# ORNL/DDStore

Measured on AMD Instinct MI355X. Metric: samples/sec (global-shuffle sample fetch), higher is better.
Workload: dtype bf16; 1 GPU; model=store-globalshuffle-fetch, global_batch=262144, rows_per_rank=2097152, row_bytes=512, store_dtype=f32, parallelism=dp1, mode=fetch

## Files before the change

### ddstore_amd/csrc/ddstore_kernels.hip

```cpp

#include "ddstore_kernels.h"

#include <hip/hip_fp16.h>
#include <hip/hip_bf16.h>
#include <hip/hip_fp8.h>
#include <type_traits>
#include <cstdlib>
#include <string>

namespace ddstore {

namespace {

constexpr int kBlock = 256;
constexpr int64_t kMaxBlocks = 32768;

inline int n_blocks(int64_t work_items) {
    int64_t b = (work_items + kBlock - 1) / kBlock;
    if (b < 1) b = 1;
    if (b > kMaxBlocks) b = kMaxBlocks;
    return (int)b;
}

template <typename T, int N>
struct alignas(sizeof(T) * N) VecT {
    T v[N];
};

__device__ __forceinline__ int owner_of(const int64_t* prefix, int nparts, int64_t row) {
    int lo = 0, hi = nparts - 1;
    while (lo < hi) {
        int mid = (lo + hi + 1) >> 1;
        if (prefix[mid] <= row) lo = mid; else hi = mid - 1;
    }
    return lo;
}

template <typename P, int NPFX = 1>
struct LdsDir {
    int64_t prefix[NPFX][DDS_MAX_PARTS + 1];
    P base[DDS_MAX_PARTS];

    __device__ __forceinline__ void load(const void* const* peer_base, int nparts,
                                         const int64_t* gprefix0,
                                         const int64_t* gprefix1 = nullptr) {
        for (int i = threadIdx.x; i <= nparts; i += kBlock) {
            prefix[0][i] = gprefix0[i];
            if constexpr (NPFX == 2) prefix[1][i] = gprefix1[i];
        }
        for (int i = threadIdx.x; i < nparts; i += kBlock)
            base[i] = reinterpret_cast<P>(peer_base[i]);
        __syncthreads();
    }
};

template <typename P, int NPFX>
__device__ __forceinline__ int owner_of(const LdsDir<P, NPFX>& d, int nparts, int64_t row) {
    return owner_of(d.prefix[0], nparts, row);
}

template <typename P, int NPFX>
__device__ __forceinline__ bool out_of_range(const LdsDir<P, NPFX>& d, int nparts,
                                             int64_t g) {
    return g < 0 || g >= d.prefix[0][nparts];
}

template <typename T>
constexpr bool is_fp8_v =
    std::is_same_v<T, __hip_fp8_e4m3> || std::is_same_v<T, __hip_fp8_e5m2>;

__device__ __forceinline__ float f64_to_f32(double v) {
#pragma clang fp contract(off)
    return static_cast<float>(v);
}

template <typename Tout, typename Tin>
__device__ __forceinline__ Tout cvt(Tin v) {
    if constexpr (std::is_same_v<Tout, Tin>) {
        return v;
    } else if constexpr (std::is_same_v<Tin, double> &&
                         (std::is_same_v<Tout, __half> ||
                          std::is_same_v<Tout, __hip_bfloat16>)) {
        return cvt<Tout, float>(f64_to_f32(v));
    } else if constexpr (std::is_same_v<Tout, uint8_t> &&
                         std::is_floating_point_v<Tin>) {
        return static_cast<uint8_t>(static_cast<int32_t>(v));
    } else if constexpr (std::is_same_v<Tin, __half>) {
        return cvt<Tout, float>(__half2float(v));
    } else if constexpr (std::is_same_v<Tin, __hip_bfloat16>) {
        return cvt<Tout, float>(__bfloat162float(v));
    } else if constexpr (is_fp8_v<Tin>) {
        return cvt<Tout, float>(static_cast<float>(v));
    } else if constexpr (std::is_same_v<Tout, __half>) {
        return __float2half(static_cast<float>(v));
    } else if constexpr (std::is_same_v<Tout, __hip_bfloat16>) {
        return __float2bfloat16(static_cast<float>(v));
    } else if constexpr (is_fp8_v<Tout>) {
        const float f = static_cast<float>(v);
        Tout r(f);
        if constexpr (std::is_same_v<Tout, __hip_fp8_e4m3>) {
            if (fabsf(f) > 464.0f) r.__x = 0x7F;
        } else {
            if (fabsf(f) >= 61440.0f) r.__x = f < 0.0f ? 0xFC : 0x7C;
        }
        return r;
    } else {
        return static_cast<Tout>(v);
    }
}

struct XfIdentity {
    static constexpr bool kNeedsCol = false;
    template <typename Tout, typename Tin>
    __device__ __forceinline__ Tout apply(Tin v) const { return v; }
};
struct XfCast {
    static constexpr bool kNeedsCol = false;
    template <typename Tout, typename Tin>
    __device__ __forceinline__ Tout apply(Tin v) const { return cvt<Tout>(v); }
};
struct XfAffine {
    static constexpr bool kNeedsCol = false;
    float scale, shift;
    uint32_t opaque_zero = 0;
    template <typename Tout, typename Tin>
    __device__ __forceinline__ Tout apply(Tin v) const {
        float y = fmaf(cvt<float>(v), scale, shift);
        if constexpr (std::is_same_v<Tout, __half>)
            y = __uint_as_float(__float_as_uint(y) | opaque_zero);
        return cvt<Tout>(y);
    }
};
struct XfAffineCol {
    static constexpr bool kNeedsCol = true;
    const float* scale;
    const float* shift;
    uint32_t opaque_zero = 0;
    template <typename Tout, typename Tin>
    __device__ __forceinline__ Tout apply(Tin v, float sc, float sh) const {
        float y = fmaf(cvt<float>(v), sc, sh);
        if constexpr (std::is_same_v<Tout, __half>)
            y = __uint_as_float(__float_as_uint(y) | opaque_zero);
        return cvt<Tout>(y);
    }
};

template <typename Tout, int VEC, bool CONTIG, typename Xf, typename Tin>
__device__ __forceinline__ void xf_chunk(const Xf& xf, const float* sc, const float* sh,
                                         const VecT<Tin, VEC>& vin, VecT<Tout, VEC>& vout,
                                         uint32_t col0, uint32_t disp = 0) {
    if constexpr (!Xf::kNeedsCol) {
#pragma unroll
        for (int k = 0; k < VEC; ++k) vout.v[k] = xf.template apply<Tout>(vin.v[k]);
    } else if constexpr (CONTIG) {
        const VecT<float, VEC> s = *reinterpret_cast<const VecT<float, VEC>*>(sc + col0);
        const VecT<float, VEC> h = *reinterpret_cast<const VecT<float, VEC>*>(sh + col0);
#pragma unroll
        for (int k = 0; k < VEC; ++k)
            vout.v[k] = xf.template apply<Tout>(vin.v[k], s.v[k], h.v[k]);
    } else {
        uint32_t cc = col0;
#pragma unroll
        for (int k = 0; k < VEC; ++k) {
            vout.v[k] = xf.template apply<Tout>(vin.v[k], sc[cc], sh[cc]);
            cc = cc + 1 == disp ? 0 : cc + 1;
        }
    }
}

template <typename Tin, typename Tout, int VEC, typename Xf>
__global__ void __launch_bounds__(kBlock)
k_gather_oneshot(const void* const* peer_base, const int64_t* gprefix, int nparts,
                 const int64_t* idx, int64_t nidx, int64_t row_elems, Xf xf,
                 Tout* __restrict__ out, unsigned long long* oob) {
    using Vin = VecT<Tin, VEC>;
    using Vout = VecT<Tout, VEC>;
    __shared__ LdsDir<const Tin*> dir;
    dir.load(peer_base, nparts, gprefix);

    const int64_t cpr = row_elems / VEC;
    const int64_t total = nidx * cpr;
    for (int64_t t = (int64_t)blockIdx.x * kBlock + threadIdx.x; t < total;
         t += (int64_t)gridDim.x * kBlock) {
        const int64_t r = t / cpr;
        const int64_t c = t - r * cpr;
        const int64_t g = idx[r];
        if (out_of_range(dir, nparts, g)) {
            if (c == 0) atomicAdd(oob, 1ull);
            continue;
        }
        const int p = owner_of(dir, nparts, g);
        const Vin vin = *reinterpret_cast<const Vin*>(
            dir.base[p] + (g - dir.prefix[0][p]) * row_elems + c * VEC);
        Vout vout;
        if constexpr (Xf::kNeedsCol)
            xf_chunk<Tout, VEC, true>(xf, xf.scale, xf.shift, vin, vout,
                                      (uint32_t)c * VEC);
        else
            xf_chunk<Tout, VEC, true>(xf, nullptr, nullptr, vin, vout, 0u);
        *reinterpret_cast<Vout*>(out + t * VEC) = vout;
    }
}

typedef uint32_t dds_u32x4 __attribute__((ext_vector_type(4)));
typedef uint32_t dds_u32x2 __attribute__((ext_vector_type(2)));
#define DDS_GLOBAL_AS __attribute__((address_space(1)))

template <typename V>
__device__ __forceinline__ void store_out(V* p, const V& v) {
    static_assert(sizeof(V) == 16, "store side is exactly 16 B per lane");
    dds_u32x4 w;
    __builtin_memcpy(&w, &v, 16);
    __builtin_nontemporal_store(w, reinterpret_cast<dds_u32x4*>(p));
}

template <typename V>
__device__ __forceinline__ V load_global(uintptr_t a) {
    constexpr int B = sizeof(V);
    V r;
    if constexpr (B % 16 == 0) {
        dds_u32x4 w[B / 16];
#pragma unroll
        for (int i = 0; i < B / 16; ++i)
            w[i] = ((const DDS_GLOBAL_AS dds_u32x4*)a)[i];
        __builtin_memcpy(&r, w, B);
    } else if constexpr (B == 8) {
        const dds_u32x2 w = *(const DDS_GLOBAL_AS dds_u32x2*)a;
        __builtin_memcpy(&r, &w, B);
    } else if constexpr (B == 4) {
        const uint32_t w = *(const DDS_GLOBAL_AS uint32_t*)a;
        __builtin_memcpy(&r, &w, B);
    } else {
        static_assert(B == 2, "unsupported vector size");
        const uint16_t w = *(const DDS_GLOBAL_AS uint16_t*)a;
        __builtin_memcpy(&r, &w, B);
    }
    return r;
}

template <int INB>
constexpr int tiled_unroll() {
    return INB >= 128 ? 1 : (128 / INB > 8 ? 8 : 128 / INB);
}

template <typename Xf, int VEC, int U, bool = Xf::kNeedsCol>
struct TiledCols {};
template <typename Xf, int VEC, int U>
struct TiledCols<Xf, VEC, U, true> {
    VecT<float, VEC> s[U], h[U];
};

template <typename Tin, typename Tout, typename Xf, bool LDSDIR>
__global__ void __launch_bounds__(kBlock)
k_gather_tiled(const GatherDirK dir, const void* const* peer_base,
               const int64_t* gprefix, int nparts,
               const int64_t* __restrict__ idx, int64_t nidx, int64_t ntiles,
               uint32_t cpr, uint32_t tile_rows, Xf xf,
               Tout* __restrict__ out, unsigned long long* oob) {
    constexpr int VEC = 16 / sizeof(Tout);
    constexpr int INB = VEC * sizeof(Tin);
    constexpr int U = tiled_unroll<INB>();
    using Vin = VecT<Tin, VEC>;
    using Vout = VecT<Tout, VEC>;
    __shared__ LdsDir<uintptr_t> ldir;
    if constexpr (LDSDIR) ldir.load(peer_base, nparts, gprefix);
    const int64_t total = LDSDIR ? ldir.prefix[0][nparts] : dir.prefix[DDS_DIR_KPARTS];
    TiledCols<Xf, VEC, U> tc;

    const uint32_t lane = threadIdx.x & 63;
    const uint32_t wave = __builtin_amdgcn_readfirstlane(threadIdx.x >> 6);
    const int64_t wstride = (int64_t)gridDim.x * (kBlock / 64);
    int64_t tile = (int64_t)blockIdx.x * (kBlock / 64) + wave;
    if (tile >= ntiles) return;

    const uint32_t q64 = 64u / cpr, r64 = 64u % cpr;
    const uint32_t rl0 = lane / cpr, c0 = lane - rl0 * cpr;
    const int64_t row_bytes = (int64_t)cpr * INB;

    int64_t g_next = 0;
    {
        const int64_t r = tile * tile_rows + lane;
        if (lane < tile_rows && r < nidx) g_next = idx[r];
    }
    for (; tile < ntiles; tile += wstride) {
        const int64_t row0 = tile * tile_rows;
        const int64_t left = nidx - row0;
        const uint32_t nrows = left < (int64_t)tile_rows ? (uint32_t)left : tile_rows;
        const int64_t g = g_next;
        if (tile + wstride < ntiles) {
            const int64_t r = (tile + wstride) * tile_rows + lane;
            if (lane < tile_rows && r < nidx) g_next = idx[r];
        }
        uintptr_t src = 0;
        if (lane < nrows) {
            if (g < 0 || g >= total) {
                atomicAdd(oob, 1ull);
            } else if constexpr (LDSDIR) {
                const int p = owner_of(ldir, nparts, g);
                src = ldir.base[p] + (uintptr_t)((g - ldir.prefix[0][p]) * row_bytes);
            } else {
                int64_t pf = dir.prefix[0];
                uintptr_t bs = reinterpret_cast<uintptr_t>(dir.base[0]);
#pragma unroll
                for (int k = 1; k < DDS_DIR_KPARTS; ++k) {
                    const bool ge = dir.prefix[k] <= g;
                    pf = ge ? dir.prefix[k] : pf;
                    bs = ge ? reinterpret_cast<uintptr_t>(dir.base[k]) : bs;
                }
                src = bs + (uintptr_t)((g - pf) * row_bytes);
            }
        }
        Vout* __restrict__ op = reinterpret_cast<Vout*>(out) + row0 * cpr;
        const uint32_t nch = nrows * cpr;
        const bool clean = __ballot(lane < nrows && src == 0) == 0;
        uint32_t rl = rl0, c = c0;
        for (uint32_t jb = 0; jb < nch; jb += 64u * U) {
            if (clean && jb + 64u * U <= nch) {
                Vin vin[U];
#pragma unroll
                for (int u = 0; u < U; ++u) {
                    const uintptr_t sp =
                        (uintptr_t)__shfl((unsigned long long)src, (int)(rl & 63u));
                    if constexpr (Xf::kNeedsCol) {
                        tc.s[u] = *reinterpret_cast<const VecT<float, VEC>*>(xf.scale + c * VEC);
                        tc.h[u] = *reinterpret_cast<const VecT<float, VEC>*>(xf.shift + c * VEC);
                    }
                    vin[u] = load_global<Vin>(sp + (uintptr_t)(c * (uint32_t)INB));
                    c += r64;
                    rl += q64;
                    if (c >= cpr) {
                        c -= cpr;
                        rl += 1;
                    }
                }
#pragma unroll
                for (int u = 0; u < U; ++u) {
                    Vout vout;
                    if constexpr (Xf::kNeedsCol) {
#pragma unroll
                        for (int k = 0; k < VEC; ++k)
                            vout.v[k] = xf.template apply<Tout>(vin[u].v[k], tc.s[u].v[k],
                                                                tc.h[u].v[k]);
                    } else {
#pragma unroll
                        for (int k = 0; k < VEC; ++k)
                            vout.v[k] = xf.template apply<Tout>(vin[u].v[k]);
                    }
                    store_out(&op[jb + 64u * u + lane], vout);
                }
            } else {
#pragma unroll 1
                for (int u = 0; u < U; ++u) {
                    const uint32_t j = jb + 64u * u + lane;
                    const uintptr_t sp =
                        (uintptr_t)__shfl((unsigned long long)src, (int)(rl & 63u));
                    if (j < nch && sp != 0) {
                        const Vin v =
                            load_global<Vin>(sp + (uintptr_t)(c * (uint32_t)INB));
                        Vout vout;
                        if constexpr (Xf::kNeedsCol) {
                            xf_chunk<Tout, VEC, true>(xf, xf.scale, xf.shift, v, vout,
                                                      c * (uint32_t)VEC);
                        } else {
#pragma unroll
                            for (int k = 0; k < VEC; ++k)
                                vout.v[k] = xf.template apply<Tout>(v.v[k]);
                        }
                        store_out(&op[j], vout);
                    }
                    c += r64;
                    rl += q64;
                    if (c >= cpr) {
                        c -= cpr;
                        rl += 1;
                    }
                }
            }
        }
    }
}

__global__ void __launch_bounds__(kBlock)
k_csr_lens(const int64_t* goff, const int64_t* idx, int64_t nidx, int64_t nsamples,
           int64_t* __restrict__ lens, unsigned long long* oob,
           unsigned long long* elems) {
    int64_t acc = 0;
    for (int64_t i = (int64_t)blockIdx.x * kBlock + threadIdx.x; i < nidx;
         i += (int64_t)gridDim.x * kBlock) {
        const int64_t g = idx[i];
        if (g < 0 || g >= nsamples) {
            lens[i] = 0;
            if (oob) atomicAdd(oob, 1ull);
            continue;
        }
        const int64_t L = goff[g + 1] - goff[g];
        lens[i] = L;
        acc += L;
    }
    if (elems) {
        for (int off = 32; off > 0; off >>= 1) acc += __shfl_down(acc, off);
        if ((threadIdx.x & 63) == 0 && acc)
            atomicAdd(elems, (unsigned long long)acc);
    }
}

__device__ __forceinline__ void copy_dwords_store16(
    uint32_t* __restrict__ dst, const uint32_t* __restrict__ src,
    int64_t nd, int tid, int nthreads) {
    const int64_t h_align = (int64_t)((4 - ((((uintptr_t)dst) >> 2) & 3)) & 3);
    const int64_t h = h_align < nd ? h_align : nd;
    for (int64_t i = tid; i < h; i += nthreads) dst[i] = src[i];
    const int64_t nb = (nd - h) >> 2;
    uint4* d4 = reinterpret_cast<uint4*>(dst + h);
    const uint32_t* s2 = src + h;
    for (int64_t i = tid; i < nb; i += nthreads) {
        uint4 o;
        o.x = s2[4 * i];
        o.y = s2[4 * i + 1];
        o.z = s2[4 * i + 2];
        o.w = s2[4 * i + 3];
        d4[i] = o;
    }
    for (int64_t i = h + (nb << 2) + tid; i < nd; i += nthreads) dst[i] = src[i];
}

template <typename U>
__device__ __forceinline__ void copy_units(U* dst, const U* src, int64_t n, int tid,
                                           int nthreads) {
    if constexpr (std::is_same_v<U, uint32_t>) {
        copy_dwords_store16(dst, src, n, tid, nthreads);
    } else {
        for (int64_t c = tid; c < n; c += nthreads) dst[c] = src[c];
    }
}

template <typename U, int GROUP>
__global__ void __launch_bounds__(kBlock)
k_gather_csr_wave(const void* const* peer_base,
                  const int64_t* sample_prefix, const int64_t* elem_prefix, int nparts,
                  const int64_t* goff,
                  const int64_t* idx, int64_t nidx,
                  const int64_t* out_off, int64_t units_per_elem,
                  int64_t cap_elems,
                  U* __restrict__ out, unsigned long long* ctrs) {
    __shared__ LdsDir<const U*, 2> dir;
    dir.load(peer_base, nparts, sample_prefix, elem_prefix);

    constexpr int GPB = kBlock / GROUP;
    const int64_t first = (int64_t)blockIdx.x * GPB + threadIdx.x / GROUP;
    const int64_t step = (int64_t)gridDim.x * GPB;
    const int tid = threadIdx.x % GROUP;
    for (int64_t s = first; s < nidx; s += step) {
        const int64_t g = idx[s];
        if (out_of_range(dir, nparts, g)) {
            if (tid == 0) atomicAdd(ctrs + DDS_CTR_OOB, 1ull);
            continue;
        }
        const int p = owner_of(dir, nparts, g);
        const int64_t e0 = goff[g];
        const int64_t len = goff[g + 1] - e0;
        const int64_t o0 = out_off[s];
        if (len <= 0) continue;
        if (o0 < 0 || o0 + len > cap_elems) {
            if (tid == 0) {
                atomicAdd(ctrs + DDS_CTR_CAP, 1ull);
                atomicAdd(ctrs + DDS_CTR_ELEMS,
                          (unsigned long long)(-(long long)len));
            }
            continue;
        }
        copy_units<U>(out + o0 * units_per_elem,
                      dir.base[p] + (e0 - dir.prefix[1][p]) * units_per_elem,
                      len * units_per_elem, tid, GROUP);
    }
}

constexpr int kItemBytes = 1024;

__device__ __forceinline__ void block_scan_pair(int64_t& x, int64_t& y,
                                                int64_t* s_wsum2, int lane,
                                                int wave, int64_t* tile_tot) {
    for (int off = 1; off < 64; off <<= 1) {
        int64_t ax = __shfl_up(x, off);
        int64_t ay = __shfl_up(y, off);
        if (lane >= off) {
            x += ax;
            y += ay;
        }
    }
    if (lane == 63) {
        s_wsum2[2 * wave] = x;
        s_wsum2[2 * wave + 1] = y;
    }
    __syncthreads();
    if (threadIdx.x == 0) {
        int64_t ax = 0, ay = 0;
        for (int w = 0; w < kBlock / 64; ++w) {
            int64_t tx = s_wsum2[2 * w], ty = s_wsum2[2 * w + 1];
            s_wsum2[2 * w] = ax;
            s_wsum2[2 * w + 1] = ay;
            ax += tx;
            ay += ty;
        }
        if (tile_tot) {
            tile_tot[0] = ax;
            tile_tot[1] = ay;
        }
    }
    __syncthreads();
    x += s_wsum2[2 * wave];
    y += s_wsum2[2 * wave + 1];
}

__global__ void __launch_bounds__(kBlock)
k_csr_plan1(const int64_t* goff, int64_t nsamples,
            const int64_t* idx, int64_t nidx, int64_t item_elems,
            int64_t* __restrict__ lens_tmp, int64_t* __restrict__ e0_tmp,
            int64_t* __restrict__ aggs, unsigned long long* ctrs) {
    __shared__ int64_t s_wsum2[2 * (kBlock / 64)];
    __shared__ int64_t s_tot[2];
    const int lane = threadIdx.x & 63;
    const int wave = threadIdx.x >> 6;
    const int64_t ntiles = (nidx + kBlock - 1) / kBlock;
    for (int64_t tile = blockIdx.x; tile < ntiles; tile += gridDim.x) {
        const int64_t i = tile * kBlock + threadIdx.x;
        int64_t L = 0, e0 = -1;
        if (i < nidx) {
            const int64_t g = idx[i];
            if (g < 0 || g >= nsamples) {
                atomicAdd(ctrs + DDS_CTR_OOB, 1ull);
            } else {
                e0 = goff[g];
                L = goff[g + 1] - e0;
            }
            lens_tmp[i] = L;
            e0_tmp[i] = e0;
        }
        int64_t x = L;
        int64_t y = L > 0 ? (L + item_elems - 1) / item_elems : 0;
        block_scan_pair(x, y, s_wsum2, lane, wave, s_tot);
        if (threadIdx.x == 0) {
            aggs[2 * tile] = s_tot[0];
            aggs[2 * tile + 1] = s_tot[1];
        }
        __syncthreads();
    }
}

__global__ void __launch_bounds__(kBlock)
k_csr_plan2(int64_t* __restrict__ aggs, int64_t ntiles,
            int64_t* __restrict__ meta, unsigned long long* ctrs) {
    __shared__ int64_t s_wsum2[2 * (kBlock / 64)];
    __shared__ int64_t s_tot[2];
    __shared__ int64_t s_carry[2];
    const int lane = threadIdx.x & 63;
    const int wave = threadIdx.x >> 6;
    if (threadIdx.x == 0) {
        s_carry[0] = 0;
        s_carry[1] = 0;
    }
    __syncthreads();
    for (int64_t base = 0; base < ntiles; base += kBlock) {
        const int64_t t = base + threadIdx.x;
        int64_t x = t < ntiles ? aggs[2 * t] : 0;
        int64_t y = t < ntiles ? aggs[2 * t + 1] : 0;
        const int64_t mx = x, my = y;
        block_scan_pair(x, y, s_wsum2, lane, wave, s_tot);
        if (t < ntiles) {
            aggs[2 * t] = s_carry[0] + x - mx;
            aggs[2 * t + 1] = s_carry[1] + y - my;
        }
        __syncthreads();
        if (threadIdx.x == 0) {
            s_carry[0] += s_tot[0];
            s_carry[1] += s_tot[1];
        }
        __syncthreads();
    }
    if (threadIdx.x == 0) {
        meta[0] = s_carry[1];
        meta[1] = s_carry[0];
        atomicAdd(ctrs + DDS_CTR_ELEMS, (unsigned long long)s_carry[0]);
    }
}

static_assert(DDS_MAX_PARTS <= 128,
              "the owner travels as p << 56 in a signed 64-bit descriptor and comes "
              "back as (int)(d0 >> 56): 127 is the largest owner that keeps it "
              "non-negative");
__global__ void __launch_bounds__(kBlock)
k_csr_plan3(const int64_t* __restrict__ lens_tmp,
            const int64_t* __restrict__ e0_tmp, int64_t nidx,
            const int64_t* sample_prefix, const int64_t* elem_prefix,
            int nparts, const int64_t* idx,
            int64_t item_elems, int64_t units_per_elem, int64_t cap_elems,
            const int64_t* __restrict__ aggs,
            int64_t* __restrict__ out_off,
            int64_t* __restrict__ desc, int64_t desc_cap,
            unsigned long long* ctrs) {
    __shared__ int64_t s_wsum2[2 * (kBlock / 64)];
    __shared__ int64_t s_sprefix[DDS_MAX_PARTS + 1];
    __shared__ int64_t s_eprefix[DDS_MAX_PARTS + 1];
    for (int i = threadIdx.x; i <= nparts; i += kBlock) {
        s_sprefix[i] = sample_prefix[i];
        s_eprefix[i] = elem_prefix[i];
    }
    __syncthreads();
    const int lane = threadIdx.x & 63;
    const int wave = threadIdx.x >> 6;
    const int64_t ntiles = (nidx + kBlock - 1) / kBlock;
    for (int64_t tile = blockIdx.x; tile < ntiles; tile += gridDim.x) {
        const int64_t i = tile * kBlock + threadIdx.x;
        const int64_t L = i < nidx ? lens_tmp[i] : 0;
        int64_t x = L;
        int64_t items = L > 0 ? (L + item_elems - 1) / item_elems : 0;
        int64_t y = items;
        block_scan_pair(x, y, s_wsum2, lane, wave, nullptr);
        const int64_t e_base = aggs[2 * tile], i_base = aggs[2 * tile + 1];
        if (i < nidx) {
            const int64_t excl_e = e_base + x - L;
            const int64_t excl_i = i_base + y - items;
            out_off[i + 1] = e_base + x;
            if (i == 0) out_off[0] = 0;
            if (L > 0) {
                if (excl_e + L > cap_elems ||
                    excl_i + items > desc_cap ||
                    L * units_per_elem >= (int64_t(1) << 44)) {
                    atomicAdd(ctrs + DDS_CTR_CAP, 1ull);
                    atomicAdd(ctrs + DDS_CTR_ELEMS,
                              (unsigned long long)(-(long long)L));
                    const int64_t end =
                        items < desc_cap - excl_i ? excl_i + items : desc_cap;
                    for (int64_t j = excl_i; j < end; ++j) {
                        desc[2 * j] = 0;
                        desc[2 * j + 1] = 0;
                    }
                } else {
                    const int64_t g = idx[i];
                    const int64_t p = owner_of(s_sprefix, nparts, g);
                    const int64_t src0 =
                        (e0_tmp[i] - s_eprefix[p]) * units_per_elem;
                    const int64_t dst0 = excl_e * units_per_elem;
                    const int64_t iu = item_elems * units_per_elem;
                    const int64_t nu = L * units_per_elem;
                    for (int64_t k = 0; k < items; ++k) {
                        const int64_t off = k * iu;
                        const int64_t n = nu - off < iu ? nu - off : iu;
                        desc[2 * (excl_i + k)] = (p << 56) | (src0 + off);
                        desc[2 * (excl_i + k) + 1] = (n << 44) | (dst0 + off);
                    }
                }
            }
        }
        __syncthreads();
    }
}

template <typename U, int GROUP>
__global__ void __launch_bounds__(kBlock)
k_gather_csr_items(const void* const* peer_base, int nparts,
                   const int64_t* __restrict__ desc,
                   const int64_t* __restrict__ meta, int64_t desc_cap,
                   U* __restrict__ out) {
    __shared__ const U* s_base[DDS_MAX_PARTS];
    for (int i = threadIdx.x; i < nparts; i += kBlock)
        s_base[i] = reinterpret_cast<const U*>(peer_base[i]);
    __syncthreads();
    const int64_t total = meta[0] < desc_cap ? meta[0] : desc_cap;
    constexpr int GPB = kBlock / GROUP;
    const int64_t first = (int64_t)blockIdx.x * GPB + threadIdx.x / GROUP;
    const int64_t step = (int64_t)gridDim.x * GPB;
    const int tid = threadIdx.x % GROUP;
    for (int64_t j = first; j < total; j += step) {
        const int64_t d0 = desc[2 * j];
        const int64_t d1 = desc[2 * j + 1];
        const int p = (int)(d0 >> 56);
        const int64_t src_u = d0 & ((int64_t(1) << 56) - 1);
        const int64_t n_u = d1 >> 44;
        const int64_t dst_u = d1 & ((int64_t(1) << 44) - 1);
        copy_units<U>(out + dst_u, s_base[p] + src_u, n_u, tid, GROUP);
    }
}

constexpr int kPadCountBlocks = 64;

template <typename P>
__device__ __forceinline__ void count_padded(const LdsDir<P, 2>& dir, int nparts,
                                             const int64_t* goff, const int64_t* idx,
                                             int64_t nidx, int64_t max_len,
                                             unsigned long long* s_acc,
                                             unsigned long long* ctrs) {
    const int64_t nb = gridDim.x < (unsigned)kPadCountBlocks ? gridDim.x : kPadCountBlocks;
    unsigned long long acc_elems = 0, acc_oob = 0;
    for (int64_t i = (int64_t)blockIdx.x * kBlock + threadIdx.x; i < nidx;
         i += nb * kBlock) {
        const int64_t g = idx[i];
        if (out_of_range(dir, nparts, g)) {
            acc_oob += 1;
        } else {
            const int64_t len = goff[g + 1] - goff[g];
            acc_elems += (unsigned long long)(len < max_len ? len : max_len);
        }
    }
    for (int off = 32; off > 0; off >>= 1) {
        acc_elems += __shfl_down(acc_elems, off);
        acc_oob += __shfl_down(acc_oob, off);
    }
    if ((threadIdx.x & 63) == 0) {
        s_acc[2 * (threadIdx.x >> 6)] = acc_elems;
        s_acc[2 * (threadIdx.x >> 6) + 1] = acc_oob;
    }
    __syncthreads();
    if (threadIdx.x == 0) {
        unsigned long long e = 0, o = 0;
        for (int w = 0; w < kBlock / 64; ++w) {
            e += s_acc[2 * w];
            o += s_acc[2 * w + 1];
        }
        if (e) atomicAdd(ctrs + DDS_CTR_ELEMS, e);
        if (o) atomicAdd(ctrs + DDS_CTR_OOB, o);
    }
}

template <typename Tin, typename Tout, int VEC, typename Xf>
__global__ void __launch_bounds__(kBlock)
k_gather_csr_padded(const void* const* peer_base, const int64_t* sample_prefix,
                    const int64_t* elem_prefix, int nparts, const int64_t* goff,
                    const int64_t* idx, int64_t nidx, int64_t disp, int64_t max_len,
                    int lg_group, bool aligned, Xf xf, dds_u32x4 pad16,
                    Tout* __restrict__ out, int64_t* __restrict__ lengths,
                    unsigned long long* ctrs) {
    using Vin = VecT<Tin, VEC>;
    using Vout = VecT<Tout, VEC>;
    static_assert(sizeof(Vout) <= 16, "pad16 covers one output chunk");
    __shared__ LdsDir<const Tin*, 2> dir;
    __shared__ unsigned long long s_acc[2 * (kBlock / 64)];
    dir.load(peer_base, nparts, sample_prefix, elem_prefix);

    Vout vpad;
    __builtin_memcpy(&vpad, &pad16, sizeof(Vout));
    const int group = 1 << lg_group;
    const int tid = threadIdx.x & (group - 1);
    const int64_t first =
        (int64_t)blockIdx.x * (kBlock >> lg_group) + (threadIdx.x >> lg_group);
    const int64_t step = (int64_t)gridDim.x * (kBlock >> lg_group);
    const int64_t row_elems = max_len * disp;
    const int64_t cpr = row_elems / VEC;
    const float* csc = nullptr;
    const float* csh = nullptr;
    uint32_t d32 = 0, col0 = 0, cstep = 0;
    if constexpr (Xf::kNeedsCol) {
        csc = xf.scale;
        csh = xf.shift;
        d32 = (uint32_t)disp;
        col0 = (uint32_t)(((uint32_t)tid * (uint32_t)VEC) % d32);
        cstep = (uint32_t)(((uint32_t)group * (uint32_t)VEC) % d32);
    }
    if (blockIdx.x < kPadCountBlocks)
        count_padded(dir, nparts, goff, idx, nidx, max_len, s_acc, ctrs);
    for (int64_t s = first; s < nidx; s += step) {
        const int64_t g = idx[s];
        const Tin* sp = nullptr;
        int64_t nvalid = 0;
        if (out_of_range(dir, nparts, g)) {
            if (tid == 0) lengths[s] = 0;
        } else {
            const int p = owner_of(dir, nparts, g);
            const int64_t e0 = goff[g];
            const int64_t len = goff[g + 1] - e0;
            const int64_t take = len < max_len ? len : max_len;
            sp = dir.base[p] + (e0 - dir.prefix[1][p]) * disp;
            nvalid = take * disp;
            if (tid == 0) lengths[s] = len;
        }
        Vout* __restrict__ op = reinterpret_cast<Vout*>(out + s * row_elems);
        uint32_t col = col0;
        for (int64_t c = tid; c < cpr; c += group) {
            const int64_t e = c * VEC;
            Vout vout = vpad;
            if (e < nvalid) {
                if (VEC == 1 || aligned) {
                    const Vin vin = *reinterpret_cast<const Vin*>(sp + e);
                    xf_chunk<Tout, VEC, true>(xf, csc, csh, vin, vout, col);
                } else if (e + VEC <= nvalid) {
                    Vin x;
#pragma unroll
                    for (int k = 0; k < VEC; ++k) x.v[k] = sp[e + k];
                    xf_chunk<Tout, VEC, false>(xf, csc, csh, x, vout, col, d32);
                } else {
                    uint32_t cc = col;
#pragma unroll
                    for (int k = 0; k < VEC; ++k) {
                        if (e + k < nvalid) {
                            if constexpr (Xf::kNeedsCol)
                                vout.v[k] = xf.template apply<Tout>(sp[e + k], csc[cc],
                                                                    csh[cc]);
                            else
                                vout.v[k] = xf.template apply<Tout>(sp[e + k]);
                        }
                        if constexpr (Xf::kNeedsCol) cc = cc + 1 == d32 ? 0 : cc + 1;
                    }
                }
            }
            op[c] = vout;
            if constexpr (Xf::kNeedsCol) {
                col += cstep;
                if (col >= d32) col -= d32;
            }
        }
    }
}


__global__ void __launch_bounds__(kBlock)
k_csr_scan3(const int64_t* __restrict__ lens_tmp, int64_t nidx,
            const int64_t* __restrict__ aggs, int64_t* __restrict__ out_off) {
    __shared__ int64_t s_wsum2[2 * (kBlock / 64)];
    const int lane = threadIdx.x & 63;
    const int wave = threadIdx.x >> 6;
    const int64_t ntiles = (nidx + kBlock - 1) / kBlock;
    for (int64_t tile = blockIdx.x; tile < ntiles; tile += gridDim.x) {
        const int64_t i = tile * kBlock + threadIdx.x;
        int64_t x = i < nidx ? lens_tmp[i] : 0;
        int64_t y = 0;
        block_scan_pair(x, y, s_wsum2, lane, wave, nullptr);
        if (i < nidx) {
            out_off[i + 1] = aggs[2 * tile] + x;
            if (i == 0) out_off[0] = 0;
        }
        __syncthreads();
    }
}

template <typename T>
struct IdPair {
    T src, dst;
};

constexpr int kGraphGroup = 64;

template <typename Tin, typename Tout, int GROUP, bool COO>
__global__ void __launch_bounds__(kBlock)
k_gather_csr_relabel(const void* const* peer_base, const int64_t* sample_prefix,
                     const int64_t* elem_prefix, int nparts, const int64_t* goff,
                     const int64_t* idx, int64_t nidx,
                     const int64_t* __restrict__ ptr,
                     const int64_t* __restrict__ edge_ptr, int64_t ncap,
                     int64_t ecap, Tout* __restrict__ out,
                     unsigned long long* ctrs) {
    using Pin = VecT<Tin, 2>;
    __shared__ LdsDir<const Pin*, 2> dir;
    dir.load(peer_base, nparts, sample_prefix, elem_prefix);

    constexpr int GPB = kBlock / GROUP;
    const int64_t first = (int64_t)blockIdx.x * GPB + threadIdx.x / GROUP;
    const int64_t step = (int64_t)gridDim.x * GPB;
    const int tid = threadIdx.x % GROUP;
    for (int64_t s = first; s < nidx; s += step) {
        const int64_t g = idx[s];
        if (out_of_range(dir, nparts, g)) continue;
        const int64_t o0 = edge_ptr[s];
        const int64_t len = edge_ptr[s + 1] - o0;
        if (len <= 0) continue;
        if (ptr[s + 1] > ncap || o0 < 0 || o0 + len > ecap) {
            if (tid == 0) {
                atomicAdd(ctrs + DDS_CTR_CAP, 1ull);
                atomicAdd(ctrs + DDS_CTR_ELEMS, (unsigned long long)(-(long long)len));
            }
            continue;
        }
        const Tout shift = static_cast<Tout>(ptr[s]);
        const int p = owner_of(dir, nparts, g);
        const Pin* __restrict__ sp = dir.base[p] + (goff[g] - dir.prefix[1][p]);
        for (int64_t e = tid; e < len; e += GROUP) {
            const Pin v = sp[e];
            const Tout a = static_cast<Tout>(v.v[0]) + shift;
            const Tout b = static_cast<Tout>(v.v[1]) + shift;
            if constexpr (COO) {
                out[o0 + e] = a;
                out[ecap + o0 + e] = b;
            } else {
                reinterpret_cast<IdPair<Tout>*>(out)[o0 + e] = IdPair<Tout>{a, b};
            }
        }
    }
}

template <typename T>
__device__ __forceinline__ void fill_store16(T* __restrict__ dst, int64_t n, T val,
                                             int64_t tid, int64_t nthreads) {
    constexpr int V = 16 / sizeof(T);
    using Vt = VecT<T, V>;
    const int64_t h_align =
        (int64_t)(((16 - ((uintptr_t)dst & 15)) & 15) / sizeof(T));
    const int64_t h = h_align < n ? h_align : n;
    for (int64_t i = tid; i < h; i += nthreads) dst[i] = val;
    const int64_t nb = (n - h) / V;
    Vt vv;
#pragma unroll
    for (int k = 0; k < V; ++k) vv.v[k] = val;
    Vt* d = reinterpret_cast<Vt*>(dst + h);
    for (int64_t i = tid; i < nb; i += nthreads) d[i] = vv;
    for (int64_t i = h + nb * V + tid; i < n; i += nthreads) dst[i] = val;
}

__device__ __forceinline__ int64_t block_last_le(const int64_t* __restrict__ a,
                                                 int64_t n, int64_t cap) {
    int64_t lo = 0, hi = n;
    while (hi > lo) {
        const int64_t m = hi - lo + 1;
        const int64_t stride = (m + kBlock - 1) / kBlock;
        const int64_t q = lo + (int64_t)threadIdx.x * stride;
        const int c = __syncthreads_count(q <= hi && a[q] <= cap);
        const int64_t nlo = lo + (int64_t)(c - 1) * stride;
        const int64_t nhi = nlo + stride - 1;
        lo = nlo;
        hi = nhi < hi ? nhi : hi;
    }
    return lo;
}

template <typename Tout, int GROUP>
__global__ void __launch_bounds__(kBlock)
k_graph_fill(const int64_t* __restrict__ ptr, const int64_t* __restrict__ edge_ptr,
             int64_t nidx, int64_t ncap, int64_t ecap, bool coo, Tout fill,
             int64_t* __restrict__ batch, Tout* __restrict__ edge_out) {
    const int64_t kn = block_last_le(ptr, nidx, ncap);
    const int64_t ke_all = block_last_le(edge_ptr, nidx, ecap);
    const int64_t ke = ke_all < kn ? ke_all : kn;
    const int64_t node_end = ptr[kn];
    const int64_t edge_end = edge_ptr[ke];

    constexpr int GPB = kBlock / GROUP;
    const int tid = threadIdx.x % GROUP;
    for (int64_t s = (int64_t)blockIdx.x * GPB + threadIdx.x / GROUP; s < kn;
         s += (int64_t)gridDim.x * GPB) {
        const int64_t o0 = ptr[s];
        fill_store16<int64_t>(batch + o0, ptr[s + 1] - o0, s, tid, GROUP);
    }
    const int64_t gt = (int64_t)blockIdx.x * kBlock + threadIdx.x;
    const int64_t nt = (int64_t)gridDim.x * kBlock;
    fill_store16<int64_t>(batch + node_end, ncap - node_end, nidx, gt, nt);
    if (coo) {
        fill_store16<Tout>(edge_out + edge_end, ecap - edge_end, fill, gt, nt);
        fill_store16<Tout>(edge_out + ecap + edge_end, ecap - edge_end, fill, gt, nt);
    } else {
        fill_store16<Tout>(edge_out + 2 * edge_end, 2 * (ecap - edge_end), fill, gt, nt);
    }
}

template <typename V>
__global__ void __launch_bounds__(kBlock)
k_scatter_rows(V* __restrict__ base, int64_t nrows, int64_t chunks_per_row,
               const int64_t* local_idx, int64_t nidx,
               const V* __restrict__ src, unsigned long long* oob) {
    const int64_t total = nidx * chunks_per_row;
    for (int64_t t = (int64_t)blockIdx.x * kBlock + threadIdx.x; t < total;
         t += (int64_t)gridDim.x * kBlock) {
        const int64_t r = t / chunks_per_row;
        const int64_t c = t - r * chunks_per_row;
        const int64_t l = local_idx[r];
        if (l < 0 || l >= nrows) {
            if (c == 0) atomicAdd(oob, 1ull);
            continue;
        }
        base[l * chunks_per_row + c] = src[t];
    }
}

template <typename T>
constexpr int stat_vec() {
    return sizeof(T) == 1 ? 8 : 16 / (int)sizeof(T);
}

template <typename T>
__device__ __forceinline__ double stat_f64(T v) {
    if constexpr (std::is_same_v<T, __half>) return (double)__half2float(v);
    else if constexpr (std::is_same_v<T, __hip_bfloat16>) return (double)__bfloat162float(v);
    else if constexpr (is_fp8_v<T>) return (double)static_cast<float>(v);
    else return (double)v;
}

template <typename T>
// ... 672 lines not shown
```

Measured before the change: 6.814 billion samples/s.

## Batch-load copy chunks with clamped addresses and prefetch gather descriptors

Replaces the dword copy loop with one that issues K 16-byte-worth loads per thread up front, using clamped (always-valid) addresses and an asm pin so all loads are in flight before the stores. Head and tail dwords are loaded unconditionally from a safe pointer to avoid divergent branches. The items kernel now loads its first descriptor and meta before the LDS base setup and barrier, and software-prefetches the next descriptor. This adds register pressure and redundant clamped loads, and uses 32-bit index math that assumes sub-2^31 dword extents.

```diff
diff --git a/ddstore_amd/csrc/csr_copy.h b/ddstore_amd/csrc/csr_copy.h
--- /dev/null
+++ b/ddstore_amd/csrc/csr_copy.h
@@ -0,0 +1,95 @@
+#pragma once
+
+#include <cstdint>
+
+#if defined(__HIPCC__)
+#define DDS_COPY_HD __host__ __device__ __forceinline__
+#else
+#define DDS_COPY_HD inline
+#endif
+
+namespace ddstore {
+
+constexpr int kCsrCopyChunks = 4;
+
+DDS_COPY_HD void csr_copy_pin(uint32_t& v) {
+#if defined(__HIP_DEVICE_COMPILE__)
+    asm volatile("" : "+v"(v));
+#else
+    (void)v;
+#endif
+}
+
+typedef uint32_t csr_copy_u32x4 __attribute__((vector_size(16)));
+
+DDS_COPY_HD uint32_t csr_copy_bound32(int64_t x) {
+    return x < 0x7fffffff ? (uint32_t)x : 0x7fffffffu;
+}
+
+template <int K>
+DDS_COPY_HD void csr_copy_load_chunks(uint32_t (&v)[K][4], const uint32_t* s4,
+                                      uint32_t lim, uint32_t o0, int nthreads) {
+#pragma unroll
+    for (int k = 0; k < K; ++k) {
+        const uint32_t i = o0 + 4u * (uint32_t)(k * nthreads);
+        const uint32_t* p = s4 + (i < lim ? i : lim);
+        v[k][0] = p[0];
+        v[k][1] = p[1];
+        v[k][2] = p[2];
+        v[k][3] = p[3];
+    }
+#pragma unroll
+    for (int k = 0; k < K; ++k) {
+        csr_copy_pin(v[k][0]);
+        csr_copy_pin(v[k][1]);
+        csr_copy_pin(v[k][2]);
+        csr_copy_pin(v[k][3]);
+    }
+}
+
+template <int K>
+DDS_COPY_HD void csr_copy_store_chunks(const uint32_t (&v)[K][4], uint32_t* d,
+                                       uint32_t nb, int tid, int nthreads) {
+#pragma unroll
+    for (int k = 0; k < K; ++k) {
+        if ((uint32_t)(tid + k * nthreads) < nb) {
+            const csr_copy_u32x4 o = {v[k][0], v[k][1], v[k][2], v[k][3]};
+            *reinterpret_cast<csr_copy_u32x4*>(d + 4 * (k * nthreads)) = o;
+        }
+    }
+}
+
+template <int K = kCsrCopyChunks>
+DDS_COPY_HD void copy_dwords_store16(uint32_t* __restrict__ dst,
+                                     const uint32_t* __restrict__ src,
+                                     const uint32_t* __restrict__ safe16,
+                                     int64_t nd, int tid, int nthreads) {
+    const int h_align = (int)((4 - ((((uintptr_t)dst) >> 2) & 3)) & 3);
+    const int h = h_align < nd ? h_align : (int)nd;
+    const int64_t nb = (nd - h) >> 2;
+    const int64_t t0 = h + (nb << 2);
+    const uint32_t* s1 = nd > 0 ? src : safe16;
+    const int64_t last1 = nd > 0 ? nd - 1 : 0;
+    const uint32_t* s4 = nd >= 4 ? src : safe16;
+    const int64_t last4 = nd >= 4 ? nd - 4 : 0;
+    const int64_t step = (int64_t)K * nthreads;
+    const uint32_t o0 = (uint32_t)(h + 4 * tid);
+    uint32_t* d = dst + o0;
+
+    uint32_t hv = s1[tid < last1 ? tid : last1];
+    uint32_t tv = s1[t0 + tid < last1 ? t0 + tid : last1];
+    uint32_t v[K][4];
+    csr_copy_load_chunks<K>(v, s4, csr_copy_bound32(last4), o0, nthreads);
+    csr_copy_pin(hv);
+    csr_copy_pin(tv);
+    if (tid < h) dst[tid] = hv;
+    csr_copy_store_chunks<K>(v, d, csr_copy_bound32(nb), tid, nthreads);
+    if (t0 + tid < nd) dst[t0 + tid] = tv;
+    for (int64_t c0 = step; c0 < nb; c0 += step) {
+        csr_copy_load_chunks<K>(v, s4 + 4 * c0, csr_copy_bound32(last4 - 4 * c0), o0,
+                                nthreads);
+        csr_copy_store_chunks<K>(v, d + 4 * c0, csr_copy_bound32(nb - c0), tid, nthreads);
+    }
+}
+
+}
diff --git a/ddstore_amd/csrc/ddstore_kernels.hip b/ddstore_amd/csrc/ddstore_kernels.hip
--- a/ddstore_amd/csrc/ddstore_kernels.hip
+++ b/ddstore_amd/csrc/ddstore_kernels.hip
@@ -1,5 +1,6 @@
 
 #include "ddstore_kernels.h"
+#include "csr_copy.h"
 
 #include <hip/hip_fp16.h>
 #include <hip/hip_bf16.h>
@@ -404,31 +405,12 @@
     }
 }
 
-__device__ __forceinline__ void copy_dwords_store16(
-    uint32_t* __restrict__ dst, const uint32_t* __restrict__ src,
-    int64_t nd, int tid, int nthreads) {
-    const int64_t h_align = (int64_t)((4 - ((((uintptr_t)dst) >> 2) & 3)) & 3);
-    const int64_t h = h_align < nd ? h_align : nd;
-    for (int64_t i = tid; i < h; i += nthreads) dst[i] = src[i];
-    const int64_t nb = (nd - h) >> 2;
-    uint4* d4 = reinterpret_cast<uint4*>(dst + h);
-    const uint32_t* s2 = src + h;
-    for (int64_t i = tid; i < nb; i += nthreads) {
-        uint4 o;
-        o.x = s2[4 * i];
-        o.y = s2[4 * i + 1];
-        o.z = s2[4 * i + 2];
-        o.w = s2[4 * i + 3];
-        d4[i] = o;
-    }
-    for (int64_t i = h + (nb << 2) + tid; i < nd; i += nthreads) dst[i] = src[i];
-}
-
 template <typename U>
-__device__ __forceinline__ void copy_units(U* dst, const U* src, int64_t n, int tid,
-                                           int nthreads) {
+__device__ __forceinline__ void copy_units(U* dst, const U* src, const void* safe16,
+                                           int64_t n, int tid, int nthreads) {
     if constexpr (std::is_same_v<U, uint32_t>) {
-        copy_dwords_store16(dst, src, n, tid, nthreads);
+        copy_dwords_store16(dst, src, reinterpret_cast<const uint32_t*>(safe16), n, tid,
+                            nthreads);
     } else {
         for (int64_t c = tid; c < n; c += nthreads) dst[c] = src[c];
     }
@@ -470,7 +452,7 @@
             continue;
         }
         copy_units<U>(out + o0 * units_per_elem,
-                      dir.base[p] + (e0 - dir.prefix[1][p]) * units_per_elem,
+                      dir.base[p] + (e0 - dir.prefix[1][p]) * units_per_elem, goff + g,
                       len * units_per_elem, tid, GROUP);
     }
 }
@@ -663,22 +645,30 @@
                    const int64_t* __restrict__ meta, int64_t desc_cap,
                    U* __restrict__ out) {
     __shared__ const U* s_base[DDS_MAX_PARTS];
-    for (int i = threadIdx.x; i < nparts; i += kBlock)
-        s_base[i] = reinterpret_cast<const U*>(peer_base[i]);
-    __syncthreads();
-    const int64_t total = meta[0] < desc_cap ? meta[0] : desc_cap;
     constexpr int GPB = kBlock / GROUP;
     const int64_t first = (int64_t)blockIdx.x * GPB + threadIdx.x / GROUP;
     const int64_t step = (int64_t)gridDim.x * GPB;
     const int tid = threadIdx.x % GROUP;
-    for (int64_t j = first; j < total; j += step) {
-        const int64_t d0 = desc[2 * j];
-        const int64_t d1 = desc[2 * j + 1];
-        const int p = (int)(d0 >> 56);
+    const int64_t* slot = desc + 2 * (first < desc_cap - 1 ? first : desc_cap - 1);
+    int64_t d0 = slot[0];
+    int64_t d1 = slot[1];
+    const int64_t m0 = meta[0];
+    for (int i = threadIdx.x; i < nparts; i += kBlock)
+        s_base[i] = reinterpret_cast<const U*>(peer_base[i]);
+    __syncthreads();
+    const int64_t total = m0 < desc_cap ? m0 : desc_cap;
+    for (int64_t j = first; j < total;) {
+        const int64_t n_u = d1 >> 44;
+        const int p = n_u > 0 ? (int)(d0 >> 56) : 0;
         const int64_t src_u = d0 & ((int64_t(1) << 56) - 1);
-        const int64_t n_u = d1 >> 44;
         const int64_t dst_u = d1 & ((int64_t(1) << 44) - 1);
-        copy_units<U>(out + dst_u, s_base[p] + src_u, n_u, tid, GROUP);
+        copy_units<U>(out + dst_u, s_base[p] + src_u, slot, n_u, tid, GROUP);
+        j += step;
+        if (j < total) {
+            slot = desc + 2 * j;
+            d0 = slot[0];
+            d1 = slot[1];
+        }
     }
 }
 
```

After: 6.812 billion samples/s, median of 2. No clear change (-0.0%).
